# yvette256/nerfstudio-thermal

Hardware: AMD Instinct MI355X
Metric: train rays/sec (4096-ray batch, 96 samples/ray) (higher is better)
Workload: dtype f32; 1 GPU; thermal-nerfacto density_mode=shared train step (pixel sampling+raygen+fwd+losses+bwd+allreduce+Adam), 4096 rays/GPU, 256/96 proposal + 48 field samples, hash 16x2^19x2 + 2x(5x2^17x2), 8 cameras (4 RGB + 4 thermal); rays_per_gpu=4096, parallelism=dp1, grad_scaler=device-side (optim.DeviceGradScaler)

## Files before the change

nerfstudio-thermal_amd/csrc/tn_field_dpos.h:

```cpp
#pragma once
#include "tn_common.h"

struct DposArgs {
  const float* origins; const float* directions; const float* e_bins; const float* g_enc; const float* jac;
  int64_t N; int S; int L; int64_t PT;
  float* d_origins; float* d_directions;
  float* cam_bias; uint32_t* fin_counter; const float* hw0; const float* emb; float* gemb; float* ghw0; int num_images;
};

__device__ __forceinline__ void emb_finish_jobs(float* __restrict__ cam_bias, uint32_t* __restrict__ counter, const float* __restrict__ hw0,
                                                const float* __restrict__ emb, float* __restrict__ gemb, float* __restrict__ ghw0, int num_images,
                                                float* sums , int* flag , unsigned bid, unsigned nblk) {
  const int t = threadIdx.x;
  const int njobs = num_images + 8;
  if ((int)bid >= njobs) return;
  const unsigned workers = (unsigned)njobs < nblk ? (unsigned)njobs : nblk;
  for (int job = bid; job < njobs; job += nblk) {
    if (job < num_images) {
      const int cam = job;
      float v = 0.0f;
      if (t < 64) {
        v = cam_bias[(int64_t)cam * 64 + t];
        sums[t] = v;
      }
      __syncthreads();
      if (t < 64 && __ballot(v != 0.0f) != 0ull) {
        const int e = t & 31, half = t >> 5;
        float a = 0.0f;
        for (int f = 0; f < 32; ++f) a += hw0[(32 * half + f) * 63 + 31 + e] * sums[32 * half + f];
        a += __shfl_xor(a, 32, 64);
        if (half == 0 && a != 0.0f) gemb[(int64_t)cam * 32 + e] += a;
      }
      __syncthreads();
    } else {
      const int o = (job - num_images) * 256 + t;
      if (t < 256 && o < 2048) {
        const int f = o >> 5, e = o & 31;
        float a = 0.0f;
        for (int cam = 0; cam < num_images; ++cam) {
          const float b = cam_bias[(int64_t)cam * 64 + f];
          if (b != 0.0f) a += b * emb[(int64_t)cam * 32 + e];
        }
        if (a != 0.0f) ghw0[f * 63 + 31 + e] += a;
      }
    }
  }
  __syncthreads();
  if (t == 0) *flag = (__hip_atomic_fetch_add(counter, 1u, __ATOMIC_RELAXED, __HIP_MEMORY_SCOPE_AGENT) == workers - 1) ? 1 : 0;
  __syncthreads();
  if (*flag) {
    for (int i = t; i < num_images * 64; i += blockDim.x) cam_bias[i] = 0.0f;
    if (t == 0) *counter = 0u;
  }
}

__device__ __forceinline__ void field_dpos_body(const DposArgs& a, unsigned bid, unsigned nblk, float* emb_sums , int* emb_flag) {
  if (a.cam_bias != nullptr) emb_finish_jobs(a.cam_bias, a.fin_counter, a.hw0, a.emb, a.gemb, a.ghw0, a.num_images, emb_sums, emb_flag, bid, nblk);
  const int64_t N = a.N, PT = a.PT;
  const int S = a.S, L = a.L;
  const int64_t P = N * (int64_t)S;
  const int64_t ntiles = tn_cdiv(P, 32);
  const int lane = threadIdx.x & 63, j = lane & 31, h = lane >> 5;
  typedef float v2f_t __attribute__((ext_vector_type(2)));
  for (int64_t tile = (int64_t)bid * (blockDim.x >> 6) + (threadIdx.x >> 6); tile < ntiles; tile += (int64_t)nblk * (blockDim.x >> 6)) {
    const int64_t p = tile * 32 + j;
    const bool live = p < P;
    const int64_t pc = live ? p : P - 1;
    float dx = 0.f, dy = 0.f, dz = 0.f;
#pragma unroll
    for (int q = 0; q < 4; ++q) {
      float2 gl[2];
      v2f_t jl[2][3];
#pragma unroll
      for (int e = 0; e < 2; ++e) {
        const int l = 4 * q + 2 * h + e;
        if (l < L) {
          gl[e] = *reinterpret_cast<const float2*>(a.g_enc + (int64_t)l * 2 * P + 2 * pc);
          const v2f_t* jp = reinterpret_cast<const v2f_t*>(a.jac) + (int64_t)l * 3 * PT + pc;
#pragma unroll
          for (int k = 0; k < 3; ++k) jl[e][k] = __builtin_nontemporal_load(jp + k * PT);
        } else {
          gl[e] = make_float2(0.f, 0.f);
#pragma unroll
          for (int k = 0; k < 3; ++k) jl[e][k] = v2f_t{0.f, 0.f};
        }
      }
      dx += gl[0].x * jl[0][0].x + gl[0].y * jl[0][0].y + gl[1].x * jl[1][0].x + gl[1].y * jl[1][0].y;
      dy += gl[0].x * jl[0][1].x + gl[0].y * jl[0][1].y + gl[1].x * jl[1][1].x + gl[1].y * jl[1][1].y;
      dz += gl[0].x * jl[0][2].x + gl[0].y * jl[0][2].y + gl[1].x * jl[1][2].x + gl[1].y * jl[1][2].y;
    }
    dx += __shfl_xor(dx, 32, 64); dy += __shfl_xor(dy, 32, 64); dz += __shfl_xor(dz, 32, 64);
    const int64_t ray = tn_div_index(pc, S, P);
    const int s = (int)(pc - ray * S);
    const float* o = a.origins + ray * 3;
    const float* d = a.directions + ray * 3;
    const float* eb = a.e_bins + ray * (S + 1) + s;
    const float st = eb[0], en = eb[1];
    const Contracted c = tn_contract(o[0], o[1], o[2], d[0], d[1], d[2], st, en);
    float wx, wy, wz;
    tn_contract_bwd(c, dx, dy, dz, wx, wy, wz);
    if (!live || h != 0) { wx = wy = wz = 0.0f; }
    const float tm = (st + en) / 2.0f;
    float v[6] = {wx, wy, wz, wx * tm, wy * tm, wz * tm};
    const int r32 = (int)ray;
    const int prev = __shfl_up(r32, 1, 64);
    const bool head = (j == 0) || (prev != r32);
    const unsigned long long H = __ballot(head);
    const int start = 63 - __clzll(H & (~0ull >> (63 - lane)));
    const bool tail = (j == 31) || ((H >> (lane + 1)) & 1ull);
#pragma unroll
// ... 16 lines not shown
```

nerfstudio-thermal_amd/csrc/tn_scatter.hip:

```cpp
#include "tn_common.h"
#include "tn_field_dpos.h"
#include "tn_pose_finish.h"
#include "tn_adam.h"
#include <float.h>
#include <stdlib.h>
#include <stdio.h>
#include <vector>
#include <algorithm>

__device__ __forceinline__ float seg_sum4(float v, int start, int lane) {
  int sl = lane >> 2;
#pragma unroll
  for (int o = 1; o < 16; o <<= 1) {
    float t = __shfl_up(v, 4 * o, 64);
    if (sl - o >= start) v += t;
  }
  return v;
}

__global__ void __launch_bounds__(256) k_grid_scatter(GridK g, const float* __restrict__ origins, const float* __restrict__ directions,
                                                      const float* __restrict__ e_bins, const float* __restrict__ g_enc, int ld, int64_t N, int S,
                                                      float* __restrict__ d_origins, float* __restrict__ d_directions, int level_groups, ReplicaK rk) {
  const bool want_dpos = d_origins != nullptr;
  const int lane = tn_lane();
// ... 554 lines not shown
  for (uint32_t blk = begin + wave * 512; blk < end; blk += FOLD_THREADS * 8) {
    nxt.ok = 0;
    if (blk + FOLD_THREADS * 8 < end) fold_load(ip, vp, blk + FOLD_THREADS * 8 + 2 * lane, end, nxt);
    FOLD_FIRE(cur)
    cur = nxt;
  }
#undef FOLD_FIRE
  __syncthreads();
  if (bk.trace && threadIdx.x == 0) bk.trace[16 * blk + 2] = wall_clock64();
  float2* dst = g.grad + (size_t)l * g.tsize + ((size_t)sl << bk.slice_log2);
  for (uint32_t t0 = 0; t0 < slots; t0 += FOLD_THREADS * 8) {
    float2 v[8], cv[8];
    bool nz[8];
#pragma unroll
    for (int u = 0; u < 8; ++u) {
      const uint32_t t = t0 + u * FOLD_THREADS + tid;
      nz[u] = false;
      if (t < slots) {
        v[u] = make_float2((float)ax[t], (float)ay[t]);
        nz[u] = v[u].x != 0.0f || v[u].y != 0.0f;
        if (nz[u] && !split) cv[u] = store ? make_float2(0.f, 0.f) : dst[t];
      }
    }
#pragma unroll
    for (int u = 0; u < 8; ++u) {
      const uint32_t t = t0 + u * FOLD_THREADS + tid;
      if (!nz[u]) continue;
      if (!split) {
        const float2 r = make_float2(cv[u].x + v[u].x, cv[u].y + v[u].y);
        dst[t] = r;
        if (g.nonfinite != nullptr && ((r.x - r.x) + (r.y - r.y)) != 0.0f) *g.nonfinite = 1.0f;
      } else {
        if (v[u].x != 0.0f) unsafeAtomicAdd(reinterpret_cast<float*>(dst + t), v[u].x);
        if (v[u].y != 0.0f) unsafeAtomicAdd(reinterpret_cast<float*>(dst + t) + 1, v[u].y);
        if (g.nonfinite != nullptr && ((v[u].x - v[u].x) + (v[u].y - v[u].y)) != 0.0f) *g.nonfinite = 1.0f;
      }
    }
  }
  if (bk.trace) {
    __syncthreads();
    if (threadIdx.x == 0) bk.trace[16 * blk + 3] = wall_clock64();
  }
}

struct SegK {
  uint16_t* idx;
  float2* val;
  uint32_t* hdr;
  uint32_t NB;
  int slice_log2, nslices;
  uint32_t merge_mask;
  uint32_t segc;
  uint32_t chunks;
  uint32_t* wmax;
};
struct FoldAdamScal {
  float* state;
  const int32_t* skipped;
  int flag, lag_index, step, max_steps, sched_step;
  double lr, lr_final, beta1, beta2;
};
__device__ __forceinline__ void fold_adam_scalars_block(const FoldAdamScal& a, double* s_term ) {
  if ((threadIdx.x & 63) == 0 && threadIdx.x < 256) {
    const int w = threadIdx.x >> 6;
    const int sk = a.skipped ? a.skipped[a.flag] : 0;
    const int lag = (a.skipped != nullptr && a.lag_index >= 0) ? a.skipped[a.lag_index] : 0;
    const double t = a.max_steps > 0 ? adam_sched_t(a.max_steps, a.sched_step, lag) : 0.0;
    if (w < 2) s_term[w] = adam_bias_correction(w == 0 ? a.beta1 : a.beta2, a.step, sk);
    else if (a.max_steps > 0) s_term[w] = adam_log_lr_term(w == 2 ? a.lr : a.lr_final, w == 2 ? 1.0 - t : t);
  }
  __syncthreads();
  if (threadIdx.x == 0) {
    float ns, bc;
    adam_scalars_finish(s_term[0], s_term[1], a.max_steps > 0 ? exp(s_term[2] + s_term[3]) : a.lr, ns, bc);
    a.state[2] = ns;
    a.state[3] = bc;
  }
}
#define SEG_CAP (BIN_THREADS * 8)
#define SEG_REGION (SEG_CAP + TN_BIN_MAX_SLICES)
#ifndef SEG_FOLD_ABLATE
#define SEG_FOLD_ABLATE 0
#endif

template <bool WANT_DPOS>
__global__ void __launch_bounds__(BIN_THREADS, 4) k_seg_bin(GridK g, const float* __restrict__ origins, const float* __restrict__ directions,
                                                         const float* __restrict__ e_bins, const float* __restrict__ g_enc, int ld, int64_t N, int S,
                                                         float* __restrict__ d_origins, float* __restrict__ d_directions, int level_groups, SegK sk,
                                                         DposArgs cw, int cw_blocks, FoldAdamScal fs) {
  __shared__ uint32_t s_cnt[TN_BIN_MAX_SLICES];
  __shared__ uint32_t s_off[TN_BIN_MAX_SLICES + 1];
  __shared__ __attribute__((aligned(16))) uint16_t s_i16[SEG_REGION];
  __shared__ __attribute__((aligned(16))) float2 s_val[SEG_REGION];
  const unsigned bx = blockIdx.x;
  if (!WANT_DPOS && bx >= sk.NB + (unsigned)cw_blocks) {
    if (blockIdx.y == 0) fold_adam_scalars_block(fs, reinterpret_cast<double*>(s_val));
    return;
  }
  if (!WANT_DPOS && bx >= sk.NB) {
    field_dpos_body(cw, blockIdx.y * (unsigned)cw_blocks + (bx - sk.NB), (unsigned)cw_blocks * gridDim.y, reinterpret_cast<float*>(s_val),
                    reinterpret_cast<int*>(s_cnt));
    return;
  }
  const int lane = tn_lane();
  const int tid = threadIdx.x, wv = tid >> 6;
  const int ns = sk.nslices;
  const int64_t P = N * (int64_t)S;
  int64_t i = (int64_t)bx * BIN_THREADS + tid;
  const bool live = i < P;
  if (!live) i = P - 1;
  int64_t ray;
  int s;
  tn_patch_order(i, N, S, ray, s);
  const int64_t p = ray * S + s;
  const float* o = origins + ray * 3;
// ... 61 lines not shown
    if (WANT_DPOS) {
      const float2* tb = g.table + (size_t)l * g.tsize;
      float sk8[8];
#pragma unroll
      for (int k = 0; k < 8; ++k) {
        const float2 t = tb[b.idx[k] & 0xfffffu];
        sk8[k] = gv.x * t.x + gv.y * t.y;
      }
      float ax = 0.f, ay = 0.f, az = 0.f;
#pragma unroll
      for (int v = 0; v < 2; ++v)
#pragma unroll
        for (int u = 0; u < 2; ++u) {
          ax += b.wy[u] * b.wz[v] * (sk8[1 + 2 * u + 4 * v] - sk8[0 + 2 * u + 4 * v]);
          ay += b.wx[u] * b.wz[v] * (sk8[u + 2 + 4 * v] - sk8[u + 0 + 4 * v]);
          az += b.wx[u] * b.wy[v] * (sk8[u + 2 * v + 4] - sk8[u + 2 * v + 0]);
        }
      dpx += ax * res;
      dpy += ay * res;
      dpz += az * res;
    }
    float vx[8], vy[8];
#pragma unroll
    for (int k = 0; k < 8; ++k) {
      const float w = b.wx[k & 1] * b.wy[(k >> 1) & 1] * b.wz[k >> 2];
      vx[k] = w * gv.x;
      vy[k] = w * gv.y;
    }
    if (merge && b.maxlen > 1) bin_run_sums(vx, vy, lane, b);
    __syncthreads();
    if (b.emit) {
#pragma unroll
      for (int k = 0; k < 8; ++k) {
        const uint32_t pos = s_off[(b.idx[k] & 0xfffffu) >> sk.slice_log2] + (b.idx[k] >> 20);
        s_i16[pos] = (uint16_t)(b.idx[k] & smask);
        s_val[pos] = make_float2(vx[k], vy[k]);
      }
    }
    __syncthreads();
    const uint32_t total = s_off[ns];
    const size_t reg = ((size_t)l * sk.NB + bx) * SEG_REGION;
    {
      float4* __restrict__ dv = reinterpret_cast<float4*>(sk.val + reg);
      const float4* sv = reinterpret_cast<const float4*>(s_val);
      for (uint32_t j = tid; j < (total + 1) / 2; j += BIN_THREADS) dv[j] = sv[j];
      uint4* __restrict__ di = reinterpret_cast<uint4*>(sk.idx + reg);
      const uint4* si = reinterpret_cast<const uint4*>(s_i16);
      for (uint32_t j = tid; j < (total + 7) / 8; j += BIN_THREADS) di[j] = si[j];
    }
  }
  if (!WANT_DPOS && fs.state != nullptr) {
#pragma unroll
    for (int o2 = 32; o2 >= 1; o2 >>= 1) gmax = max(gmax, (uint32_t)__shfl_xor((int)gmax, o2, 64));
    if (lane == 0) sk.wmax[((size_t)blockIdx.y * sk.NB + bx) * (BIN_THREADS / 64) + wv] = gmax;
  }
  if (WANT_DPOS) {
    float wxg, wyg, wzg;
    tn_contract_bwd(c, dpx, dpy, dpz, wxg, wyg, wzg);
    if (!live) { wxg = wyg = wzg = 0.0f; }
    const float tm = (st + en) / 2.0f;
    float v[6] = {wxg, wyg, wzg, wxg * tm, wyg * tm, wzg * tm};
    const int r32 = (int)ray;
    const int lead = __shfl(r32, lane & 3, 64);
    if (__all(r32 == lead)) {
#pragma unroll
      for (int k = 0; k < 6; ++k) {
        float r = v[k];
        r += __shfl_xor(r, 4, 64);
        r += __shfl_xor(r, 8, 64);
        r += __shfl_xor(r, 16, 64);
        r += __shfl_xor(r, 32, 64);
        if (lane < 4 && r != 0.0f) atomicAdd((k < 3 ? d_origins : d_directions) + ray * 3 + (k % 3), r);
      }
    } else {
#pragma unroll
      for (int k = 0; k < 6; ++k)
        if (v[k] != 0.0f) atomicAdd((k < 3 ? d_origins : d_directions) + ray * 3 + (k % 3), v[k]);
    }
  }
}

struct FoldAdamK {
  float2 *p, *m, *v;
  const float* state;
  const float* found_inf;
  float b1, b2, omb1, omb2, eps;
};
#ifndef FOLD_ADAM_BATCH
#define FOLD_ADAM_BATCH 2
#endif
template <bool ADAM>
__global__ void __launch_bounds__(FOLD_THREADS, 8) k_seg_fold(GridK g, SegK sk, uint32_t level_begin, uint32_t grad_zero_promise, PoseFinishArgs pf,
                                                           uint32_t pf_blocks, FoldAdamK fa) {
  extern __shared__ __attribute__((aligned(16))) float s_mem[];
  if (blockIdx.x < pf_blocks) {
    if ((int)blockIdx.x < pf.total_blocks) pose_finish_body(pf, (int)blockIdx.x);
    return;
  }
  const bool fused = ADAM && fa.state[1] == TN_FOLD_ADAM_FUSED;
  if (fused && *fa.found_inf != 0.0f) return;
  const uint32_t fb = blockIdx.x - pf_blocks;
  const int tid = threadIdx.x, lane = tid & 63, wave = tid >> 6;
  const uint32_t ns = (uint32_t)sk.nslices, per_level = ns * sk.chunks;
  const uint32_t l = level_begin + fb / per_level, rel = fb % per_level;
  const uint32_t ch = rel / ns, p = rel % ns;
  const uint32_t sl = (ns % 32u == 0u) ? ((p >> 5) << 5) + ((p & 7u) << 2) + ((p >> 3) & 3u) : p;
  const uint32_t slots = 1u << sk.slice_log2;
  double* ax = reinterpret_cast<double*>(s_mem);
  double* ay = ax + slots;
  uint32_t* s_h = reinterpret_cast<uint32_t*>(s_mem + 4 * slots);
  uint32_t* s_pre = s_h + sk.segc;
  uint32_t* s_tot = s_pre + sk.segc;
  const uint32_t b0 = ch * sk.segc, nseg = min(sk.segc, sk.NB - b0);
  const uint32_t my_h = (uint32_t)tid < nseg ? sk.hdr[((size_t)l * ns + sl) * sk.NB + b0 + tid] : 0u;
  {
    float4* z = reinterpret_cast<float4*>(s_mem);
    for (uint32_t t = tid; t < slots; t += FOLD_THREADS) z[t] = make_float4(0.f, 0.f, 0.f, 0.f);
  }
  {
    const uint32_t c = ((my_h >> 16) + 1u) >> 1;
    uint32_t inc = c;
#pragma unroll
    for (int o = 1; o < 64; o <<= 1) {
      const uint32_t up = __shfl_up(inc, o, 64);
      if (lane >= o) inc += up;
    }
    if ((uint32_t)tid < nseg) { s_h[tid] = my_h; s_pre[tid] = inc - c; }
    if (lane == 63) s_tot[wave] = inc;
  }
  __syncthreads();
  uint32_t total = 0;
#pragma unroll
  for (int w = 0; w < FOLD_THREADS / 64; ++w) total += s_tot[w];
  if (total == 0 && !fused) return;
  const bool split = sk.chunks > 1;
  const bool store = grad_zero_promise && !split;
  const uint32_t avg = 2u * total / max(nseg, 1u);
  const int gw_log2 = avg >= 256 ? 6 : (avg >= 96 ? 5 : 4);
  const uint32_t gw = 1u << gw_log2, ngroups = FOLD_THREADS >> gw_log2;
  const uint32_t share = (((total + ngroups - 1) / ngroups) + gw - 1) & ~(gw - 1);
  const uint32_t r_begin = ((uint32_t)tid >> gw_log2) * share, r_end = min(total, r_begin + share);
  uint32_t rr = r_begin + ((uint32_t)tid & (gw - 1));
  const size_t lvl_base = (size_t)l * sk.NB + b0;
  uint32_t sg = 0, t = 0, cnt = 0, cnt_rec = 0;
  size_t base = 0;
  auto open_seg = [&]() {
    const uint32_t h = s_h[sg];
    cnt_rec = h >> 16;
    cnt = (cnt_rec + 1u) >> 1;
    base = (lvl_base + sg) * SEG_REGION + (h & 0xffffu);
  };
  if (r_begin < total) {
    uint32_t before = 0, w = 0;
#pragma unroll
    for (int i = 0; i < FOLD_THREADS / 64; ++i) {
      const uint32_t c = s_tot[i];
      if (i == (int)w && r_begin >= before + c) { before += c; ++w; }
    }
    const uint32_t want = r_begin - before;
    uint32_t lo = w * 64, hi = min(nseg, lo + 64);
    while (hi - lo > 1) {
      const uint32_t mid = (lo + hi) >> 1;
      if (s_pre[mid] <= want) lo = mid; else hi = mid;
    }
    sg = lo;
    open_seg();
    t = want - s_pre[sg] + ((uint32_t)tid & (gw - 1));
  }
  struct FoldRec { uint32_t idp; float4 v; bool ok; };
  auto fetch = [&](FoldRec& r) {
    r.ok = rr < r_end;
    r.idp = 0;
    r.v = make_float4(0.f, 0.f, 0.f, 0.f);
    if (r.ok) {
      while (t >= cnt) {
        t -= cnt;
        ++sg;
        open_seg();
      }
#if SEG_FOLD_ABLATE & 2
      r.idp = ((uint32_t)(base + 2 * t) & (slots - 1)) * 0x10001u;
      r.v = make_float4(1.0f, 1.0f, 1.0f, 1.0f);
#else
      r.idp = *reinterpret_cast<const uint32_t*>(sk.idx + base + 2 * (size_t)t);
      r.v = *reinterpret_cast<const float4*>(sk.val + base + 2 * (size_t)t);
#endif
// ... 53 lines not shown
          gg[u] = v4f{(float)ax[2 * q], (float)ay[2 * q], (float)ax[2 * q + 1], (float)ay[2 * q + 1]};
        }
      }
#pragma unroll
      for (int u = 0; u < FOLD_ADAM_BATCH; ++u) {
        const uint32_t q = q0 + u * FOLD_THREADS + tid;
        if (q >= pairs) continue;
        const v4u zb = __builtin_bit_cast(v4u, gg[u]) | __builtin_bit_cast(v4u, mm[u]) | __builtin_bit_cast(v4u, vv[u]);
        if ((zb.x | zb.y | zb.z | zb.w) == 0u) continue;
        float4 pp = pq[u];
        float m0 = mm[u].x, m1 = mm[u].y, m2 = mm[u].z, m3 = mm[u].w, v0 = vv[u].x, v1 = vv[u].y, v2 = vv[u].z, v3 = vv[u].w;
        adam1(pp.x, gg[u].x, m0, v0, coef);
        adam1(pp.y, gg[u].y, m1, v1, coef);
        adam1(pp.z, gg[u].z, m2, v2, coef);
        adam1(pp.w, gg[u].w, m3, v3, coef);
        p4[q] = pp;
        __builtin_nontemporal_store(v4f{m0, m1, m2, m3}, m4 + q);
        __builtin_nontemporal_store(v4f{v0, v1, v2, v3}, v4 + q);
      }
    }
    return;
  }
  float2* dst = g.grad + (size_t)l * g.tsize + ((size_t)sl << sk.slice_log2);
  for (uint32_t tt = 0; tt < slots; tt += FOLD_THREADS * 8) {
    float2 w[8], cv[8];
    bool nz[8];
#pragma unroll
    for (int u = 0; u < 8; ++u) {
      const uint32_t t = tt + u * FOLD_THREADS + tid;
      nz[u] = false;
      if (t < slots) {
        w[u] = make_float2((float)ax[t], (float)ay[t]);
        nz[u] = w[u].x != 0.0f || w[u].y != 0.0f;
        if (nz[u] && !split) cv[u] = store ? make_float2(0.f, 0.f) : dst[t];
      }
    }
#pragma unroll
    for (int u = 0; u < 8; ++u) {
      const uint32_t t = tt + u * FOLD_THREADS + tid;
      if (!nz[u]) continue;
      if (!split) {
        const float2 r = make_float2(cv[u].x + w[u].x, cv[u].y + w[u].y);
        dst[t] = r;
        if (g.nonfinite != nullptr && ((r.x - r.x) + (r.y - r.y)) != 0.0f) *g.nonfinite = 1.0f;
      } else {
        if (w[u].x != 0.0f) unsafeAtomicAdd(reinterpret_cast<float*>(dst + t), w[u].x);
        if (w[u].y != 0.0f) unsafeAtomicAdd(reinterpret_cast<float*>(dst + t) + 1, w[u].y);
        if (g.nonfinite != nullptr && ((w[u].x - w[u].x) + (w[u].y - w[u].y)) != 0.0f) *g.nonfinite = 1.0f;
      }
    }
  }
}

struct FoldAdamPrep {
  const float* grads;
  int ncheck;
  int64_t off[TN_TRAIN_STEP_MAX_RANGES], cnt[TN_TRAIN_STEP_MAX_RANGES];
  float* found_inf_flag;
  float* state;
  float limit;
  const uint32_t* wmax;
  uint32_t row_words, row_stride, rows;
};
__global__ void __launch_bounds__(1024) k_fold_adam_prepare(FoldAdamPrep a) {
  __shared__ int s_bad;
  __shared__ uint32_t s_max;
  if (threadIdx.x == 0) { s_bad = 0; s_max = 0u; }
  __syncthreads();
  bool bad = false;
  for (int k = 0; k < a.ncheck; ++k) {
    const float* base = a.grads + a.off[k];
    for (int64_t i0 = threadIdx.x; i0 < a.cnt[k]; i0 += 8 * (int64_t)blockDim.x) {
      float x[8];
#pragma unroll
      for (int u = 0; u < 8; ++u) { const int64_t i = i0 + u * (int64_t)blockDim.x; x[u] = i < a.cnt[k] ? base[i] : 0.0f; }
#pragma unroll
      for (int u = 0; u < 8; ++u) bad = bad || ((x[u] - x[u]) != 0.0f);
    }
  }
  uint32_t mx = 0u;
  for (uint32_t r = 0; r < a.rows; ++r) {
    const uint32_t* row = a.wmax + (size_t)r * a.row_stride;
    for (uint32_t i0 = threadIdx.x; i0 < a.row_words; i0 += 8 * blockDim.x) {
      uint32_t w[8];
#pragma unroll
      for (int u = 0; u < 8; ++u) { const uint32_t i = i0 + u * blockDim.x; w[u] = i < a.row_words ? row[i] : 0u; }
#pragma unroll
      for (int u = 0; u < 8; ++u) mx = max(mx, w[u]);
    }
  }
#pragma unroll
  for (int o = 32; o >= 1; o >>= 1) mx = max(mx, (uint32_t)__shfl_xor((int)mx, o, 64));
  const bool wave_bad = __any(bad);
  if ((threadIdx.x & 63) == 0) {
    if (wave_bad) s_bad = 1;
    atomicMax(&s_max, mx);
  }
  __syncthreads();
  if (threadIdx.x == 0) {
    if (s_bad) *a.found_inf_flag = 1.0f;
    const float enc_max = __uint_as_float(s_max);
    a.state[0] = enc_max;
    a.state[1] = (enc_max <= a.limit) ? TN_FOLD_ADAM_FUSED : TN_FOLD_ADAM_FELL_BACK;
  }
}

static int env_int(const char* name, int dflt, int lo, int hi) {
  const char* e = getenv(name);
  int v = e ? atoi(e) : dflt;
  return v < lo ? lo : (v > hi ? hi : v);
}
static int dense_replicas() { static int r = env_int("TN_SCATTER_REPLICAS", 16, 0, 64); return r; }

static int64_t plan_replicas(const TnGrid& grid, int64_t P, ReplicaK& rk) {
  const int64_t cap = TN_SCATTER_SCRATCH_BYTES / (int64_t)sizeof(float2);
  const int64_t T = 1ll << grid.log2_hashmap_size;
  int64_t used = 0, total = 0;
  if (dense_replicas() <= 0) return 0;
  for (int l = 0; l < grid.num_levels; ++l) {
    float r = grid.res[l];
    int64_t n = 0;
    int kind = TN_REP_NONE, R = 0;
    if (r >= 1.0f && r <= 62.0f) {
      int64_t r1 = (int64_t)ceilf(r) + 1;
      n = r1 * r1 * r1;
      R = dense_replicas();
      if (n <= T && n <= 4 * P && used + n * R <= cap) kind = TN_REP_DENSE;
    }
    if (kind == TN_REP_NONE) break;
    rk.kinds |= (uint32_t)kind << (2 * l);
    rk.n[l] = (uint32_t)n;
    rk.off[l] = (uint32_t)used;
    rk.first[l] = (uint32_t)total;
    rk.R[l] = (uint8_t)R;
    used += n * R;
    total += n;
  }
  rk.total = (uint32_t)total;
  return used;
}

static int scatter_mode() { return env_int("TN_SCATTER_MODE", 2, 0, 2); }
static bool seg_mode() { return scatter_mode() == 2; }
static int merge_res();

static int seg_plan(const TnGrid& grid, int64_t P, void* scratch, SegK& sk) {
  const int L = grid.num_levels;
  sk = SegK{};
  sk.slice_log2 = std::min(TN_BIN_SLICE_LOG2, grid.log2_hashmap_size);
  sk.nslices = 1 << (grid.log2_hashmap_size - sk.slice_log2);
  TN_REQUIRE(sk.nslices <= TN_BIN_MAX_SLICES, "tn_grid_scatter: table too large for the segmented path");
  const int64_t NB = tn_cdiv(P, BIN_THREADS);
  sk.NB = (uint32_t)NB;
  const int64_t recs = (int64_t)L * NB * SEG_REGION;
  char* base = reinterpret_cast<char*>(scratch) + 256;
  sk.val = reinterpret_cast<float2*>(base);
  sk.idx = reinterpret_cast<uint16_t*>(base + recs * 8);
  sk.hdr = reinterpret_cast<uint32_t*>(base + recs * 10);
  const int64_t hdr_end = 256 + recs * 10 + (int64_t)L * sk.nslices * NB * 4, wmax_bytes = (int64_t)TN_MAX_LEVELS * NB * (BIN_THREADS / 64) * 4;
  sk.wmax = reinterpret_cast<uint32_t*>(reinterpret_cast<char*>(scratch) + hdr_end);
  TN_REQUIRE(hdr_end + wmax_bytes <= tn_scatter_scratch_bytes(P, L), "tn_grid_scatter: segmented layout exceeds the scatter scratch");
  for (int l = 0; l < L; ++l)
    if (grid.res[l] <= (float)merge_res()) sk.merge_mask |= 1u << l;
  int64_t segc = (int64_t)L * sk.nslices >= 1024 ? 1024 : std::max<int64_t>(64, std::min<int64_t>(1024, 8 * sk.nslices));
  segc = std::min<int64_t>(segc, NB);
  segc = tn_cdiv(NB, tn_cdiv(NB, segc));
  sk.segc = (uint32_t)segc;
  sk.chunks = (uint32_t)tn_cdiv(NB, segc);
  return TN_OK;
}
static int seg_level_groups(int L, uint32_t NB) {
  int level_groups = 1;
  while (level_groups < L && (int64_t)NB * level_groups < 256 * 6) level_groups *= 2;
  return std::min(level_groups, L);
}
static int fold_chunk_sparse() { static int r = env_int("TN_SCATTER_SPARSE_CHUNK", 16384, 1024, 32768) & ~1023; return r; }
static int merge_res() { static int r = env_int("TN_SCATTER_MERGE_RES", 1 << 20, 0, 1 << 20); return r; }

static int bin_plan(const TnGrid& grid, int64_t P, void* scratch, BinK& bk, uint32_t& nblk) {
  const int L = grid.num_levels;
  bk = BinK{};
  bk.slice_log2 = std::min(TN_BIN_SLICE_LOG2, grid.log2_hashmap_size);
  bk.nslices = 1 << (grid.log2_hashmap_size - bk.slice_log2);
  TN_REQUIRE(bk.nslices <= TN_BIN_MAX_SLICES, "tn_grid_scatter: table too large for the binned path");
  const int64_t cap = (tn_bin_level_records(P) / bk.nslices) & ~7ll;
  TN_REQUIRE(cap * bk.nslices < (1ll << 32), "tn_grid_scatter: batch too large for the binned path");
  bk.cap = (uint32_t)cap;
  bk.level_stride = (uint32_t)(cap * bk.nslices);
  char* base = reinterpret_cast<char*>(scratch);
  bk.count = reinterpret_cast<uint32_t*>(base);
  bk.cstride = 1;
  const int64_t cnt_bytes = 256 + (int64_t)L * TN_BIN_MAX_SLICES * 4 * TN_BIN_COUNT_STRIDE;
  bk.val = reinterpret_cast<float2*>(base + cnt_bytes);
  bk.idx = reinterpret_cast<uint16_t*>(base + cnt_bytes + (int64_t)L * tn_bin_level_records(P) * 8);
  nblk = 0;
  for (int l = 0; l < L; ++l) {
    if (grid.res[l] <= (float)merge_res()) bk.merge_mask |= 1u << l;
    const double r1 = ceil((double)grid.res[l]) + 1.0;
    const double T = (double)(1ll << grid.log2_hashmap_size), live = std::min(r1 * r1 * r1, T);
    const bool sparse = r1 * r1 * r1 < 0.5 * T || 8.0 * (double)P > 16.0 * live;
    bk.chunk[l] = sparse ? (uint32_t)fold_chunk_sparse() : 32768u;
    bk.blk0[l] = nblk;
    nblk += (uint32_t)(bk.nslices * tn_cdiv(bk.cap, bk.chunk[l]));
  }
  bk.blk0[L] = nblk;
  return TN_OK;
}

void tn_grid_scatter_counters(const TnGrid& grid, int64_t P, void* scratch, uint32_t** ptr, int* words) {
  *ptr = nullptr;
  *words = 0;
  if (P <= 0 || !tn_grid_scatter_is_binned(grid, P, scratch)) return;
  if (seg_mode()) return;
  BinK bk;
  uint32_t nblk;
  if (bin_plan(grid, P, scratch, bk, nblk) != TN_OK) return;
  *ptr = bk.count;
  *words = grid.num_levels * bk.nslices * (int)bk.cstride;
}

int tn_grid_scatter_bin(const TnGrid& grid, const float* origins, const float* directions, const float* e_bins, const float* g_enc, int ld, int64_t N,
                        int S, float* d_origins, float* d_directions, void* scratch, hipStream_t stream, bool counters_zeroed, const DposArgs* cowork,
                        const FoldAdamHost* fold_adam) {
  const int64_t P = N * (int64_t)S;
  const int L = grid.num_levels;
  TN_REQUIRE(fold_adam == nullptr || (d_origins == nullptr && tn_fold_adam_takes(grid, P, scratch)), "tn_grid_scatter: the fold does not step this table (tn_fold_adam_takes)");
  if (seg_mode()) {
    SegK sk;
    int rc = seg_plan(grid, P, scratch, sk);
    if (rc) return rc;
    GridK gk = make_gridk(grid);
    const int blocks = (int)sk.NB;
    const int level_groups = seg_level_groups(L, sk.NB);
    TN_REQUIRE(cowork == nullptr || d_origins == nullptr, "tn_grid_scatter: co-work only beside a bin pass without a d position path of its own");
    if (d_origins != nullptr) {
      hipLaunchKernelGGL(k_seg_bin<true>, dim3(blocks, level_groups), dim3(BIN_THREADS), 0, stream, gk, origins, directions, e_bins, g_enc, ld, N, S, d_origins,
                         d_directions, level_groups, sk, DposArgs{}, 0, FoldAdamScal{});
    } else {
      int cw_blocks = 0;
      if (cowork != nullptr) {
        const int64_t tiles = tn_cdiv(cowork->N * (int64_t)cowork->S, 32);
        cw_blocks = (int)std::min<int64_t>(tn_cdiv(tn_cdiv(tiles, BIN_THREADS / 64), level_groups), 2048);
      }
      FoldAdamScal fs{};
      if (fold_adam != nullptr) {
        const FoldAdamHost& h = *fold_adam;
        fs = FoldAdamScal{h.state, h.skipped, h.flag, h.lag_index, h.step, h.max_steps, h.sched_step, h.lr, h.lr_final, h.beta1, h.beta2};
      }
      hipLaunchKernelGGL(k_seg_bin<false>, dim3(blocks + cw_blocks + (fold_adam ? 1 : 0), level_groups), dim3(BIN_THREADS), 0, stream, gk, origins, directions,
                         e_bins, g_enc, ld, N, S, d_origins, d_directions, level_groups, sk, cowork ? *cowork : DposArgs{}, cw_blocks, fs);
    }
    TN_CHECK_LAUNCH("tn_grid_scatter(bin, segmented)");
    return TN_OK;
  }
  TN_REQUIRE(cowork == nullptr, "tn_grid_scatter: co-work needs the segmented path (tn_grid_scatter_takes_cowork)");
  BinK bk;
  uint32_t nblk;
  int rc = bin_plan(grid, P, scratch, bk, nblk);
  if (rc) return rc;
  if (!counters_zeroed) {
    hipError_t e = hipMemsetAsync(bk.count, 0, (size_t)L * bk.nslices * 4 * bk.cstride, stream);
    TN_REQUIRE(e == hipSuccess, "tn_grid_scatter: memset failed: %s", hipGetErrorString(e));
  }
  GridK gk = make_gridk(grid);
  const int blocks = (int)tn_cdiv(P, BIN_THREADS);
  int level_groups = 1;
  while (level_groups < L && ((int64_t)blocks * level_groups < 256 * 6 || tn_cdiv(L, level_groups) * bk.nslices > BIN_MAX_COUNTERS)) level_groups *= 2;
  level_groups = std::min(level_groups, L);
  {
    static const int forced = env_int("TN_BIN_LEVEL_GROUPS", 0, 0, TN_MAX_LEVELS);
    if (forced > 0 && tn_cdiv(L, std::min(forced, L)) * bk.nslices <= BIN_MAX_COUNTERS) level_groups = std::min(forced, L);
  }
  if (d_origins != nullptr)
    hipLaunchKernelGGL(k_grid_bin<true>, dim3(blocks, level_groups), dim3(BIN_THREADS), 0, stream, gk, origins, directions, e_bins, g_enc, ld, N, S,
                       d_origins, d_directions, level_groups, bk);
  else
    hipLaunchKernelGGL(k_grid_bin<false>, dim3(blocks, level_groups), dim3(BIN_THREADS), 0, stream, gk, origins, directions, e_bins, g_enc, ld, N, S,
                       d_origins, d_directions, level_groups, bk);
  TN_CHECK_LAUNCH("tn_grid_scatter(bin)");
  return TN_OK;
}

int tn_grid_scatter_fold(const TnGrid& grid, int64_t P, void* scratch, int level_begin, int level_end, hipStream_t stream, const PoseFinishArgs* cowork,
                         const FoldAdamHost* fold_adam) {
  const int L = grid.num_levels;
  TN_REQUIRE(level_begin >= 0 && level_begin < level_end && level_end <= L, "tn_grid_scatter_fold: bad level range");
  TN_REQUIRE(cowork == nullptr || seg_mode(), "tn_grid_scatter_fold: co-work needs the segmented path (tn_grid_scatter_takes_cowork)");
  TN_REQUIRE(fold_adam == nullptr || (level_begin == 0 && level_end == L && fold_adam->p == grid.table && tn_fold_adam_takes(grid, P, scratch)),
             "tn_grid_scatter_fold: the fold does not step this table (tn_fold_adam_takes, the whole grid in one launch)");
  if (seg_mode()) {
    SegK sk;
    int rc = seg_plan(grid, P, scratch, sk);
    if (rc) return rc;
    GridK gk = make_gridk(grid);
    const size_t shmem = (size_t)(2u << sk.slice_log2) * sizeof(double) + (size_t)sk.segc * 8 + (FOLD_THREADS / 64) * 4;
    const int max_shmem = (int)((2u << TN_BIN_SLICE_LOG2) * sizeof(double) + 1024 * 8 + (FOLD_THREADS / 64) * 4);
    const uint32_t nblk = (uint32_t)(level_end - level_begin) * (uint32_t)sk.nslices * sk.chunks;
    const uint32_t pfb = cowork ? ((uint32_t)cowork->total_blocks + 7u) & ~7u : 0u;
    if (fold_adam != nullptr) {
      const FoldAdamHost& h = *fold_adam;
      FoldAdamPrep pr{};
      pr.grads = h.grads;
      pr.ncheck = h.ncheck;
      for (int k = 0; k < h.ncheck; ++k) { pr.off[k] = h.check_off[k]; pr.cnt[k] = h.check_cnt[k]; }
      pr.found_inf_flag = h.found_inf + h.flag;
      pr.state = h.state;
      pr.limit = FLT_MAX / (8.0f * (float)P);
      pr.wmax = sk.wmax;
      pr.row_words = sk.NB * (BIN_THREADS / 64); pr.row_stride = pr.row_words; pr.rows = (uint32_t)seg_level_groups(L, sk.NB);
      hipLaunchKernelGGL(k_fold_adam_prepare, dim3(1), dim3(1024), 0, stream, pr);
      TN_CHECK_LAUNCH("tn_grid_scatter(fold: prepare)");
      const AdamCoef c = adam_coef(0.f, 0.f, h.beta1, h.beta2, h.eps);
      FoldAdamK fa{reinterpret_cast<float2*>(h.p), reinterpret_cast<float2*>(h.m), reinterpret_cast<float2*>(h.v), h.state, h.found_inf + h.flag,
                   c.b1, c.b2, c.omb1, c.omb2, c.eps};
      (void)hipFuncSetAttribute(reinterpret_cast<const void*>(&k_seg_fold<true>), hipFuncAttributeMaxDynamicSharedMemorySize, max_shmem);
      hipLaunchKernelGGL(k_seg_fold<true>, dim3(nblk + pfb), dim3(FOLD_THREADS), shmem, stream, gk, sk, (uint32_t)level_begin, (uint32_t)(gk.grad_zero ? 1 : 0),
                         cowork ? *cowork : PoseFinishArgs{}, pfb, fa);
    } else {
      (void)hipFuncSetAttribute(reinterpret_cast<const void*>(&k_seg_fold<false>), hipFuncAttributeMaxDynamicSharedMemorySize, max_shmem);
      hipLaunchKernelGGL(k_seg_fold<false>, dim3(nblk + pfb), dim3(FOLD_THREADS), shmem, stream, gk, sk, (uint32_t)level_begin, (uint32_t)(gk.grad_zero ? 1 : 0),
                         cowork ? *cowork : PoseFinishArgs{}, pfb, FoldAdamK{});
    }
    TN_CHECK_LAUNCH("tn_grid_scatter(fold, segmented)");
    return TN_OK;
  }
  BinK bk;
  uint32_t nblk_all;
  int rc = bin_plan(grid, P, scratch, bk, nblk_all);
  if (rc) return rc;
  GridK gk = make_gridk(grid);
  const uint32_t first_block = bk.blk0[level_begin], nblk = bk.blk0[level_end] - bk.blk0[level_begin];
  const size_t shmem = (size_t)(2u << bk.slice_log2) * sizeof(double);
  (void)hipFuncSetAttribute(reinterpret_cast<const void*>(&k_grid_fold), hipFuncAttributeMaxDynamicSharedMemorySize,
                            (int)((2u << TN_BIN_SLICE_LOG2) * sizeof(double)));
  static int trace_on = env_int("TN_FOLD_TRACE", 0, 0, 1);
  static unsigned long long* trace_buf = nullptr;
  if (trace_on) {
    if (!trace_buf) (void)hipMalloc(&trace_buf, (size_t)1 << 22);
    (void)hipMemsetAsync(trace_buf, 0, (size_t)nblk_all * 128, stream);
    bk.trace = trace_buf;
  }
  hipLaunchKernelGGL(k_grid_fold, dim3(nblk), dim3(FOLD_THREADS), shmem, stream, gk, bk, first_block);
  if (trace_on) {
    std::vector<unsigned long long> h((size_t)nblk_all * 16);
    (void)hipStreamSynchronize(stream);
    (void)hipMemcpy(h.data(), trace_buf, h.size() * 8, hipMemcpyDeviceToHost);
    unsigned long long t0 = ~0ull, t1 = 0;
    for (uint32_t b = 0; b < nblk_all; ++b)
      if (h[16 * b]) { t0 = std::min(t0, h[16 * b]); t1 = std::max(t1, h[16 * b + 3]); }
    fprintf(stderr, "[fold trace] %u blocks, span %.1f us (wall clock 100 MHz)\n", nblk, (t1 - t0) / 100.0);
    if (const char* dump = getenv("TN_FOLD_TRACE_FILE")) {
      if (FILE* f = fopen(dump, "wb")) { fwrite(h.data(), 8, h.size(), f); fclose(f); }
    }
    for (int l = 0; l < L; ++l) {
      double a = 0, b2 = 0, c = 0, first = 1e30, last = 0; int n = 0;
      double st[9] = {0};
      for (uint32_t b = bk.blk0[l]; b < bk.blk0[l + 1]; ++b) {
        const unsigned long long* q = &h[16 * b];
        if (!q[0]) continue;
        ++n; a += (q[1] - q[0]) / 100.0; b2 += (q[2] - q[1]) / 100.0; c += (q[3] - q[2]) / 100.0;
        first = std::min(first, (q[0] - t0) / 100.0); last = std::max(last, (q[3] - t0) / 100.0);
        unsigned long long prev = q[1];
        for (int k = 0; k < 9; ++k) { if (q[4 + k]) { st[k] += (q[4 + k] - prev) / 100.0; prev = q[4 + k]; } }
      }
      if (n) fprintf(stderr, "  level %2d: %4d active blocks, mean us: setup %.1f passes %.1f flush %.1f; first start %.1f last end %.1f | 1st iteration: passes %.2f %.2f %.2f %.2f retries %.2f %.2f %.2f sync %.2f float-atomics %.2f\n", l, n, a / n, b2 / n, c / n, first, last,
                     st[0] / n, st[1] / n, st[2] / n, st[3] / n, st[4] / n, st[5] / n, st[6] / n, st[7] / n, st[8] / n);
    }
// ... 127 lines not shown
```

Baseline: 6.285 million rays/s.

## Fold Adam prepare kernel into bin and fold kernels

Removes the single-block k_fold_adam_prepare launch that sat between the bin and fold kernels. Its non-finite gradient check moves into extra threads of the scalar block in the bin kernel, plus an inline check on the emb/hw0 gradient updates. The encoded-max reduction now happens in two steps: per-block maxima are written in the bin kernel, and every fold block reduces them redundantly. This saves a serial single-block launch and its gap, but each fold block now does extra global reads, and the fused-or-fallback decision depends on the inf flag being visible across kernels.

After: 6.307 million rays/s (median of 4 runs). About the same (+0.3%).

```diff
diff --git a/nerfstudio-thermal_amd/csrc/tn_field_dpos.h b/nerfstudio-thermal_amd/csrc/tn_field_dpos.h
--- a/nerfstudio-thermal_amd/csrc/tn_field_dpos.h
+++ b/nerfstudio-thermal_amd/csrc/tn_field_dpos.h
@@ -6,11 +6,13 @@
   int64_t N; int S; int L; int64_t PT;
   float* d_origins; float* d_directions;
   float* cam_bias; uint32_t* fin_counter; const float* hw0; const float* emb; float* gemb; float* ghw0; int num_images;
+  float* nonfinite;
 };
 
 __device__ __forceinline__ void emb_finish_jobs(float* __restrict__ cam_bias, uint32_t* __restrict__ counter, const float* __restrict__ hw0,
                                                 const float* __restrict__ emb, float* __restrict__ gemb, float* __restrict__ ghw0, int num_images,
-                                                float* sums , int* flag , unsigned bid, unsigned nblk) {
+                                                float* sums , int* flag , unsigned bid, unsigned nblk,
+                                                float* nonfinite = nullptr) {
   const int t = threadIdx.x;
   const int njobs = num_images + 8;
   if ((int)bid >= njobs) return;
@@ -29,7 +31,11 @@
         float a = 0.0f;
         for (int f = 0; f < 32; ++f) a += hw0[(32 * half + f) * 63 + 31 + e] * sums[32 * half + f];
         a += __shfl_xor(a, 32, 64);
-        if (half == 0 && a != 0.0f) gemb[(int64_t)cam * 32 + e] += a;
+        if (half == 0 && a != 0.0f) {
+          const float r = gemb[(int64_t)cam * 32 + e] + a;
+          gemb[(int64_t)cam * 32 + e] = r;
+          if (nonfinite != nullptr && (r - r) != 0.0f) *nonfinite = 1.0f;
+        }
       }
       __syncthreads();
     } else {
@@ -41,7 +47,11 @@
           const float b = cam_bias[(int64_t)cam * 64 + f];
           if (b != 0.0f) a += b * emb[(int64_t)cam * 32 + e];
         }
-        if (a != 0.0f) ghw0[f * 63 + 31 + e] += a;
+        if (a != 0.0f) {
+          const float r = ghw0[f * 63 + 31 + e] + a;
+          ghw0[f * 63 + 31 + e] = r;
+          if (nonfinite != nullptr && (r - r) != 0.0f) *nonfinite = 1.0f;
+        }
       }
     }
   }
@@ -55,7 +65,7 @@
 }
 
 __device__ __forceinline__ void field_dpos_body(const DposArgs& a, unsigned bid, unsigned nblk, float* emb_sums , int* emb_flag) {
-  if (a.cam_bias != nullptr) emb_finish_jobs(a.cam_bias, a.fin_counter, a.hw0, a.emb, a.gemb, a.ghw0, a.num_images, emb_sums, emb_flag, bid, nblk);
+  if (a.cam_bias != nullptr) emb_finish_jobs(a.cam_bias, a.fin_counter, a.hw0, a.emb, a.gemb, a.ghw0, a.num_images, emb_sums, emb_flag, bid, nblk, a.nonfinite);
   const int64_t N = a.N, PT = a.PT;
   const int S = a.S, L = a.L;
   const int64_t P = N * (int64_t)S;
diff --git a/nerfstudio-thermal_amd/csrc/tn_scatter.hip b/nerfstudio-thermal_amd/csrc/tn_scatter.hip
--- a/nerfstudio-thermal_amd/csrc/tn_scatter.hip
+++ b/nerfstudio-thermal_amd/csrc/tn_scatter.hip
@@ -630,15 +630,35 @@
   uint32_t merge_mask;
   uint32_t segc;
   uint32_t chunks;
-  uint32_t* wmax;
+  uint32_t* bmax;
 };
 struct FoldAdamScal {
   float* state;
   const int32_t* skipped;
   int flag, lag_index, step, max_steps, sched_step;
   double lr, lr_final, beta1, beta2;
+  const float* grads;
+  float* found_inf_flag;
+  int ncheck;
+  int64_t check_off[TN_TRAIN_STEP_MAX_RANGES], check_cnt[TN_TRAIN_STEP_MAX_RANGES];
 };
 __device__ __forceinline__ void fold_adam_scalars_block(const FoldAdamScal& a, double* s_term ) {
+  if (threadIdx.x >= 256) {
+    const int64_t nt = (int64_t)blockDim.x - 256, t0 = (int64_t)threadIdx.x - 256;
+    bool bad = false;
+    for (int k = 0; k < a.ncheck; ++k) {
+      const float* base = a.grads + a.check_off[k];
+      const int64_t cnt = a.check_cnt[k];
+      for (int64_t i0 = t0; i0 < cnt; i0 += 8 * nt) {
+        float x[8];
+#pragma unroll
+        for (int u = 0; u < 8; ++u) { const int64_t i = i0 + u * nt; x[u] = i < cnt ? base[i] : 0.0f; }
+#pragma unroll
+        for (int u = 0; u < 8; ++u) bad = bad || ((x[u] - x[u]) != 0.0f);
+      }
+    }
+    if (bad) *a.found_inf_flag = 1.0f;
+  }
   if ((threadIdx.x & 63) == 0 && threadIdx.x < 256) {
     const int w = threadIdx.x >> 6;
     const int sk = a.skipped ? a.skipped[a.flag] : 0;
@@ -806,7 +826,14 @@
   if (!WANT_DPOS && fs.state != nullptr) {
 #pragma unroll
     for (int o2 = 32; o2 >= 1; o2 >>= 1) gmax = max(gmax, (uint32_t)__shfl_xor((int)gmax, o2, 64));
-    if (lane == 0) sk.wmax[((size_t)blockIdx.y * sk.NB + bx) * (BIN_THREADS / 64) + wv] = gmax;
+    if (lane == 0) s_cnt[wv] = gmax;
+    __syncthreads();
+    if (tid == 0) {
+      uint32_t m = s_cnt[0];
+#pragma unroll
+      for (int w = 1; w < BIN_THREADS / 64; ++w) m = max(m, s_cnt[w]);
+      sk.bmax[(size_t)blockIdx.y * sk.NB + bx] = m;
+    }
   }
   if (WANT_DPOS) {
     float wxg, wyg, wzg;
@@ -836,10 +863,14 @@
 
 struct FoldAdamK {
   float2 *p, *m, *v;
-  const float* state;
+  float* state;
   const float* found_inf;
   float b1, b2, omb1, omb2, eps;
+  const uint32_t* bmax;
+  uint32_t nmax;
+  float limit;
 };
+#define FOLD_MAX_WORDS 4
 #ifndef FOLD_ADAM_BATCH
 #define FOLD_ADAM_BATCH 2
 #endif
@@ -851,8 +882,6 @@
     if ((int)blockIdx.x < pf.total_blocks) pose_finish_body(pf, (int)blockIdx.x);
     return;
   }
-  const bool fused = ADAM && fa.state[1] == TN_FOLD_ADAM_FUSED;
-  if (fused && *fa.found_inf != 0.0f) return;
   const uint32_t fb = blockIdx.x - pf_blocks;
   const int tid = threadIdx.x, lane = tid & 63, wave = tid >> 6;
   const uint32_t ns = (uint32_t)sk.nslices, per_level = ns * sk.chunks;
@@ -865,8 +894,19 @@
   uint32_t* s_h = reinterpret_cast<uint32_t*>(s_mem + 4 * slots);
   uint32_t* s_pre = s_h + sk.segc;
   uint32_t* s_tot = s_pre + sk.segc;
+  uint32_t* s_max = s_tot + FOLD_THREADS / 64;
   const uint32_t b0 = ch * sk.segc, nseg = min(sk.segc, sk.NB - b0);
   const uint32_t my_h = (uint32_t)tid < nseg ? sk.hdr[((size_t)l * ns + sl) * sk.NB + b0 + tid] : 0u;
+  uint32_t mx = 0u;
+  float inf_flag = 0.0f;
+  if (ADAM) {
+    uint32_t w[FOLD_MAX_WORDS];
+#pragma unroll
+    for (int u = 0; u < FOLD_MAX_WORDS; ++u) w[u] = fa.bmax[min((uint32_t)tid + u * FOLD_THREADS, fa.nmax - 1u)];
+    inf_flag = *fa.found_inf;
+#pragma unroll
+    for (int u = 0; u < FOLD_MAX_WORDS; ++u) mx = max(mx, w[u]);
+  }
   {
     float4* z = reinterpret_cast<float4*>(s_mem);
     for (uint32_t t = tid; t < slots; t += FOLD_THREADS) z[t] = make_float4(0.f, 0.f, 0.f, 0.f);
@@ -882,10 +922,28 @@
     if ((uint32_t)tid < nseg) { s_h[tid] = my_h; s_pre[tid] = inc - c; }
     if (lane == 63) s_tot[wave] = inc;
   }
+  if (ADAM) {
+#pragma unroll
+    for (int o = 32; o >= 1; o >>= 1) mx = max(mx, (uint32_t)__shfl_xor((int)mx, o, 64));
+    if (lane == 0) s_max[wave] = mx;
+  }
   __syncthreads();
   uint32_t total = 0;
 #pragma unroll
   for (int w = 0; w < FOLD_THREADS / 64; ++w) total += s_tot[w];
+  bool fused = false;
+  if (ADAM) {
+    mx = s_max[0];
+#pragma unroll
+    for (int w = 1; w < FOLD_THREADS / 64; ++w) mx = max(mx, s_max[w]);
+    const float enc_max = __uint_as_float((uint32_t)__builtin_amdgcn_readfirstlane((int)mx));
+    fused = enc_max <= fa.limit;
+    if (fb == 0 && tid == 0) {
+      fa.state[0] = enc_max;
+      fa.state[1] = fused ? TN_FOLD_ADAM_FUSED : TN_FOLD_ADAM_FELL_BACK;
+    }
+    if (fused && inf_flag != 0.0f) return;
+  }
   if (total == 0 && !fused) return;
   const bool split = sk.chunks > 1;
   const bool store = grad_zero_promise && !split;
@@ -1045,59 +1103,6 @@
   }
 }
 
-struct FoldAdamPrep {
-  const float* grads;
-  int ncheck;
-  int64_t off[TN_TRAIN_STEP_MAX_RANGES], cnt[TN_TRAIN_STEP_MAX_RANGES];
-  float* found_inf_flag;
-  float* state;
-  float limit;
-  const uint32_t* wmax;
-  uint32_t row_words, row_stride, rows;
-};
-__global__ void __launch_bounds__(1024) k_fold_adam_prepare(FoldAdamPrep a) {
-  __shared__ int s_bad;
-  __shared__ uint32_t s_max;
-  if (threadIdx.x == 0) { s_bad = 0; s_max = 0u; }
-  __syncthreads();
-  bool bad = false;
-  for (int k = 0; k < a.ncheck; ++k) {
-    const float* base = a.grads + a.off[k];
-    for (int64_t i0 = threadIdx.x; i0 < a.cnt[k]; i0 += 8 * (int64_t)blockDim.x) {
-      float x[8];
-#pragma unroll
-      for (int u = 0; u < 8; ++u) { const int64_t i = i0 + u * (int64_t)blockDim.x; x[u] = i < a.cnt[k] ? base[i] : 0.0f; }
-#pragma unroll
-      for (int u = 0; u < 8; ++u) bad = bad || ((x[u] - x[u]) != 0.0f);
-    }
-  }
-  uint32_t mx = 0u;
-  for (uint32_t r = 0; r < a.rows; ++r) {
-    const uint32_t* row = a.wmax + (size_t)r * a.row_stride;
-    for (uint32_t i0 = threadIdx.x; i0 < a.row_words; i0 += 8 * blockDim.x) {
-      uint32_t w[8];
-#pragma unroll
-      for (int u = 0; u < 8; ++u) { const uint32_t i = i0 + u * blockDim.x; w[u] = i < a.row_words ? row[i] : 0u; }
-#pragma unroll
-      for (int u = 0; u < 8; ++u) mx = max(mx, w[u]);
-    }
-  }
-#pragma unroll
-  for (int o = 32; o >= 1; o >>= 1) mx = max(mx, (uint32_t)__shfl_xor((int)mx, o, 64));
-  const bool wave_bad = __any(bad);
-  if ((threadIdx.x & 63) == 0) {
-    if (wave_bad) s_bad = 1;
-    atomicMax(&s_max, mx);
-  }
-  __syncthreads();
-  if (threadIdx.x == 0) {
-    if (s_bad) *a.found_inf_flag = 1.0f;
-    const float enc_max = __uint_as_float(s_max);
-    a.state[0] = enc_max;
-    a.state[1] = (enc_max <= a.limit) ? TN_FOLD_ADAM_FUSED : TN_FOLD_ADAM_FELL_BACK;
-  }
-}
-
 static int env_int(const char* name, int dflt, int lo, int hi) {
   const char* e = getenv(name);
   int v = e ? atoi(e) : dflt;
@@ -1150,9 +1155,9 @@
   sk.val = reinterpret_cast<float2*>(base);
   sk.idx = reinterpret_cast<uint16_t*>(base + recs * 8);
   sk.hdr = reinterpret_cast<uint32_t*>(base + recs * 10);
-  const int64_t hdr_end = 256 + recs * 10 + (int64_t)L * sk.nslices * NB * 4, wmax_bytes = (int64_t)TN_MAX_LEVELS * NB * (BIN_THREADS / 64) * 4;
-  sk.wmax = reinterpret_cast<uint32_t*>(reinterpret_cast<char*>(scratch) + hdr_end);
-  TN_REQUIRE(hdr_end + wmax_bytes <= tn_scatter_scratch_bytes(P, L), "tn_grid_scatter: segmented layout exceeds the scatter scratch");
+  const int64_t hdr_end = 256 + recs * 10 + (int64_t)L * sk.nslices * NB * 4, bmax_bytes = (int64_t)TN_MAX_LEVELS * NB * 4;
+  sk.bmax = reinterpret_cast<uint32_t*>(reinterpret_cast<char*>(scratch) + hdr_end);
+  TN_REQUIRE(hdr_end + bmax_bytes <= tn_scatter_scratch_bytes(P, L), "tn_grid_scatter: segmented layout exceeds the scatter scratch");
   for (int l = 0; l < L; ++l)
     if (grid.res[l] <= (float)merge_res()) sk.merge_mask |= 1u << l;
   int64_t segc = (int64_t)L * sk.nslices >= 1024 ? 1024 : std::max<int64_t>(64, std::min<int64_t>(1024, 8 * sk.nslices));
@@ -1239,9 +1244,15 @@
       if (fold_adam != nullptr) {
         const FoldAdamHost& h = *fold_adam;
         fs = FoldAdamScal{h.state, h.skipped, h.flag, h.lag_index, h.step, h.max_steps, h.sched_step, h.lr, h.lr_final, h.beta1, h.beta2};
-      }
+        fs.grads = h.grads;
+        fs.found_inf_flag = h.found_inf + h.flag;
+        fs.ncheck = h.ncheck;
+        for (int k = 0; k < h.ncheck; ++k) { fs.check_off[k] = h.check_off[k]; fs.check_cnt[k] = h.check_cnt[k]; }
+      }
+      DposArgs cwa = cowork ? *cowork : DposArgs{};
+      if (fold_adam != nullptr) cwa.nonfinite = fold_adam->found_inf + fold_adam->flag;
       hipLaunchKernelGGL(k_seg_bin<false>, dim3(blocks + cw_blocks + (fold_adam ? 1 : 0), level_groups), dim3(BIN_THREADS), 0, stream, gk, origins, directions,
-                         e_bins, g_enc, ld, N, S, d_origins, d_directions, level_groups, sk, cowork ? *cowork : DposArgs{}, cw_blocks, fs);
+                         e_bins, g_enc, ld, N, S, d_origins, d_directions, level_groups, sk, cwa, cw_blocks, fs);
     }
     TN_CHECK_LAUNCH("tn_grid_scatter(bin, segmented)");
     return TN_OK;
@@ -1286,26 +1297,16 @@
     int rc = seg_plan(grid, P, scratch, sk);
     if (rc) return rc;
     GridK gk = make_gridk(grid);
-    const size_t shmem = (size_t)(2u << sk.slice_log2) * sizeof(double) + (size_t)sk.segc * 8 + (FOLD_THREADS / 64) * 4;
-    const int max_shmem = (int)((2u << TN_BIN_SLICE_LOG2) * sizeof(double) + 1024 * 8 + (FOLD_THREADS / 64) * 4);
+    const size_t shmem = (size_t)(2u << sk.slice_log2) * sizeof(double) + (size_t)sk.segc * 8 + (FOLD_THREADS / 64) * 8;
+    const int max_shmem = (int)((2u << TN_BIN_SLICE_LOG2) * sizeof(double) + 1024 * 8 + (FOLD_THREADS / 64) * 8);
     const uint32_t nblk = (uint32_t)(level_end - level_begin) * (uint32_t)sk.nslices * sk.chunks;
     const uint32_t pfb = cowork ? ((uint32_t)cowork->total_blocks + 7u) & ~7u : 0u;
     if (fold_adam != nullptr) {
       const FoldAdamHost& h = *fold_adam;
-      FoldAdamPrep pr{};
-      pr.grads = h.grads;
-      pr.ncheck = h.ncheck;
-      for (int k = 0; k < h.ncheck; ++k) { pr.off[k] = h.check_off[k]; pr.cnt[k] = h.check_cnt[k]; }
-      pr.found_inf_flag = h.found_inf + h.flag;
-      pr.state = h.state;
-      pr.limit = FLT_MAX / (8.0f * (float)P);
-      pr.wmax = sk.wmax;
-      pr.row_words = sk.NB * (BIN_THREADS / 64); pr.row_stride = pr.row_words; pr.rows = (uint32_t)seg_level_groups(L, sk.NB);
-      hipLaunchKernelGGL(k_fold_adam_prepare, dim3(1), dim3(1024), 0, stream, pr);
-      TN_CHECK_LAUNCH("tn_grid_scatter(fold: prepare)");
       const AdamCoef c = adam_coef(0.f, 0.f, h.beta1, h.beta2, h.eps);
+      TN_REQUIRE(sk.NB * (uint32_t)seg_level_groups(L, sk.NB) <= FOLD_MAX_WORDS * FOLD_THREADS, "tn_grid_scatter_fold: more block maxima than a fold block reads");
       FoldAdamK fa{reinterpret_cast<float2*>(h.p), reinterpret_cast<float2*>(h.m), reinterpret_cast<float2*>(h.v), h.state, h.found_inf + h.flag,
-                   c.b1, c.b2, c.omb1, c.omb2, c.eps};
+                   c.b1, c.b2, c.omb1, c.omb2, c.eps, sk.bmax, sk.NB * (uint32_t)seg_level_groups(L, sk.NB), FLT_MAX / (8.0f * (float)P)};
       (void)hipFuncSetAttribute(reinterpret_cast<const void*>(&k_seg_fold<true>), hipFuncAttributeMaxDynamicSharedMemorySize, max_shmem);
       hipLaunchKernelGGL(k_seg_fold<true>, dim3(nblk + pfb), dim3(FOLD_THREADS), shmem, stream, gk, sk, (uint32_t)level_begin, (uint32_t)(gk.grad_zero ? 1 : 0),
                          cowork ? *cowork : PoseFinishArgs{}, pfb, fa);
```
